# Gyeeta/gyeeta

Hardware: NVIDIA H100
Metric: events/sec aggregated (higher is better)
Workload: dtype u64

## Files before the change

gyeeta_b200/csrc/gysk_device.cuh:

```cuda
#pragma once

#include <cstdint>
#include <cuda_runtime.h>

namespace gysk {

struct HistCell { unsigned long long count; long long sum; };
static constexpr int HIST_CELLS = 16;
static constexpr int HIST_MAX_CELL = 15;

struct alignas(16) TblEntry { unsigned long long key; uint32_t slot1; uint32_t pad; };
static constexpr uint32_t SLOT_INVALID = 0xFFFFFFFFu;

struct Centroid { double mean; unsigned long long weight; };
static constexpr int TD_CAP = 256;

struct alignas(16) Bin { unsigned long long cw; unsigned long long us; };
static constexpr int NBINS = 848;
static constexpr int BIN_CNT_BITS = 27;
static constexpr unsigned long long BIN_CNT_MASK = (1ull << BIN_CNT_BITS) - 1;
static constexpr int HOT_ROW_BINS = 1024, HOT_ROW_WORDS = 2 * HOT_ROW_BINS;
static_assert(NBINS <= HOT_ROW_BINS, "a row holds every bin");
__host__ __device__ __forceinline__ uint32_t hot_word(uint32_t bin) { return ((bin & 31u) << 5) | (bin >> 5); }

struct alignas(8) SlotAux { unsigned long long act_cur, act_last, err_cur, err_last; uint32_t rtt_cur, rtt_last; };

struct alignas(16) SlotBatch { uint32_t minv, maxv, touched, hot; };
struct alignas(8) SlotState { uint8_t state, issue, issue_bits, high_bits; uint32_t nconn_active; };

struct TdHead { unsigned long long total; double minv, maxv; uint32_t n; uint32_t pad; };

struct IdTable
{
	TblEntry	*ent;
	uint32_t	mask;
	uint32_t	max_slots;
	uint32_t	*count;
	unsigned long long *slot_id;
	uint32_t	*slot_host;
	int32_t		*free_n;
	uint32_t	*free_slots;
	unsigned long long *insert_fail;
};
static constexpr unsigned long long KEY_TOMBSTONE = ~0ull;

enum { CTR_IN = 0, CTR_DROPPED, CTR_RESP, CTR_TCP, CTR_TASK, CTR_FOREIGN, CTR_NKEYS, CTR_INSERT_FAIL, CTR_NTOUCHED ,
	CTR_NLONG , CTR_NEVICT, CTR_EVICTED_TOTAL,
	CTR_NHOT , CTR_NHOT_NEXT , CTR_NWINDOW ,
	CTR_NHOSTS , CTR_TASK_NEVICT , CTR_MAX };

static constexpr uint32_t JHASH_GOLDEN = 0x9e3779b9u;
static constexpr uint32_t GY_SEED = 0xceedfeadu;
static constexpr uint32_t FLOW_SEED_A = GY_SEED;
static constexpr uint32_t FLOW_SEED_B = GY_SEED ^ 0x5bd1e995u;

__host__ __device__ __forceinline__ uint32_t jhash_2words(uint32_t a, uint32_t b, uint32_t initval)
{
	uint32_t c = initval;

	a += JHASH_GOLDEN; b += JHASH_GOLDEN;
	a -= b; a -= c; a ^= (c >> 13);
	b -= c; b -= a; b ^= (a << 8);
	c -= a; c -= b; c ^= (b >> 13);
	a -= b; a -= c; a ^= (c >> 12);
	b -= c; b -= a; b ^= (a << 16);
	c -= a; c -= b; c ^= (b >> 5);
	a -= b; a -= c; a ^= (c >> 3);
	b -= c; b -= a; b ^= (a << 10);
	c -= a; c -= b; c ^= (b >> 15);
	return c;
}

__host__ __device__ __forceinline__ uint32_t uint64_hash(unsigned long long key)
{
	return jhash_2words((uint32_t)(key & 0xFFFFFFFFu), (uint32_t)(key >> 32), GY_SEED);
}

__host__ __device__ __forceinline__ uint32_t table_hash(unsigned long long key)
{
	return (uint32_t)((key * 0x9E3779B97F4A7C15ull) >> 32);
}

// ... 99 lines not shown
__device__ __forceinline__ void red_max_s64(long long *p, long long v)
{
	asm volatile("red.global.max.s64 [%0], %1;" :: "l"(p), "l"(v) : "memory");
}

__device__ __forceinline__ void prefetch_l2(const void *p)
{
	asm volatile("prefetch.global.L2 [%0];" :: "l"(p));
}

__device__ __forceinline__ unsigned long long l2_policy_evict_first()
{
	unsigned long long pol;
	asm volatile("createpolicy.fractional.L2::evict_first.b64 %0, 1.0;" : "=l"(pol));
	return pol;
}

__device__ __forceinline__ unsigned long long l2_policy_evict_last()
{
	unsigned long long pol;
	asm volatile("createpolicy.fractional.L2::evict_last.b64 %0, 1.0;" : "=l"(pol));
	return pol;
}

__device__ __forceinline__ void red_add_u64_hint(unsigned long long *p, unsigned long long v, unsigned long long pol)
{
	asm volatile("red.global.add.L2::cache_hint.u64 [%0], %1, %2;" :: "l"(p), "l"(v), "l"(pol) : "memory");
}

__device__ __forceinline__ uint32_t ld_na_hint_u32(const uint32_t *p, unsigned long long pol)
{
	uint32_t v;
	asm volatile("ld.global.L1::no_allocate.L2::cache_hint.u32 %0, [%1], %2;" : "=r"(v) : "l"(p), "l"(pol));
	return v;
}

__device__ __forceinline__ void l2_evict_normal_line(const void *p)
{
	asm volatile("applypriority.global.L2::evict_normal [%0], 128;" :: "l"(p) : "memory");
}

__device__ __forceinline__ uint4 ld_cg_v4(const void *p)
{
	uint4 v;
	asm volatile("ld.global.v4.u32 {%0, %1, %2, %3}, [%4];" : "=r"(v.x), "=r"(v.y), "=r"(v.z), "=r"(v.w) : "l"(p));
	return v;
}

__device__ __forceinline__ uint32_t ld_volatile_u32(const uint32_t *p)
{
	uint32_t v;
	asm volatile("ld.volatile.global.u32 %0, [%1];" : "=r"(v) : "l"(p));
	return v;
}

__device__ __forceinline__ void st_volatile_u32(uint32_t *p, uint32_t v)
{
	asm volatile("st.volatile.global.u32 [%0], %1;" :: "l"(p), "r"(v) : "memory");
}

__device__ __forceinline__ uint4 table_probe_first(const IdTable &t, unsigned long long key, uint32_t &pos)
{
	pos = table_hash(key) & t.mask;
	return ld_cg_v4(&t.ent[pos]);
}

// ... 61 lines not shown
```

gyeeta_b200/csrc/gysk_engine.cu:

```cuda
#include "gysk_engine.h"
#include "gysk_state.cuh"
#include "gysk_summary.cuh"
#include "gysk_wire.h"

using namespace gysk;

namespace {

thread_local std::string g_create_error;
std::atomic<uint64_t> g_engine_uid {1};

}

namespace gysk {

int fail(gysk_engine *e, int code, const char *what, cudaError_t ce)
{
	char buf[512];

	if (ce != cudaSuccess) snprintf(buf, sizeof(buf), "%s: %s", what, cudaGetErrorString(ce));
	else snprintf(buf, sizeof(buf), "%s", what);
	if (e) {
		e->err = buf;
		if (code == GYSK_ERR_CUDA) e->sticky = true;
// ... 508 lines not shown
		A(dalloc(e, &d_q, qtab.size(), false));
		if ((ce = cudaMemcpy(d_q, qtab.data(), qtab.size() * sizeof(double), cudaMemcpyHostToDevice)) != cudaSuccess) { fail(e, GYSK_ERR_CUDA, "qtab", ce); return bail(GYSK_ERR_CUDA); }
		st.td.qtab = d_q; st.td.delta = cfg.td_compression; st.td.pad = 0;
	}
	{
		auto envl = [](const char *name, long dflt) { const char *v = getenv(name); return v ? atol(v) : dflt; };
		long rows = envl("GYSK_HOT_ROWS", 2048);
		if (rows < 0) rows = 0;
		if (rows > 65536) rows = 65536;
		if ((size_t)rows > ns) rows = (long)ns;
		st.hot_cap = (uint32_t)rows;
		st.hot_min = (uint32_t)std::max(1l, envl("GYSK_HOT_MIN", 4096));
		st.hot_max = (uint32_t)std::min<long>(0xFFFFFFFFl, std::max(1l, envl("GYSK_HOT_MAX", 0xFFFFFFFFl)));
		st.hot_bin_max = (uint32_t)std::min<long>(0xFFFFFFFFl, std::max(1l, envl("GYSK_HOT_BIN_MAX", 131072)));
		st.hot_rows = nullptr; st.hot_slot = nullptr;
		if (rows) { A(dalloc(e, &st.hot_rows, (size_t)rows * HOT_ROW_WORDS)); A(dalloc(e, &st.hot_slot, (size_t)rows)); }
	}
	const size_t nsort = sort_keys(cfg);
	tmp.nkeys = nsort;
	tmp.max_tiles = sort_tiles(nsort);
	A(dalloc(e, &tmp.keys_a, nsort, false)); A(dalloc(e, &tmp.keys_b, nsort, false));
	A(dalloc(e, &tmp.tile_status, (size_t)RADIX_MAX * tmp.max_tiles));
	tmp.epoch = &e->sort_epoch;
	A(dalloc(e, &tmp.os_ghist, (size_t)OS_GHIST_WORDS));
	{
		const size_t nmw = (size_t)TD_MERGE_MAX_SMS * TD_MERGE_CTAS_PER_SM * 4;
		const size_t nbrows = batch_rows(cfg);
		A(dalloc(e, &tmp.long_slot, nbrows, false)); A(dalloc(e, &tmp.batch_rows, nbrows * HOT_ROW_WORDS));
		A(dalloc(e, &tmp.items_scratch, nmw * NBINS, false)); A(dalloc(e, &tmp.big_scratch, nmw, false));
		const uint32_t nsm = (uint32_t)prop.multiProcessorCount;
		tmp.rec_cnt_cap = nsm * IngestShape::WARPS * IngestShape::MIN_CTAS;
		tmp.recq_cap = (uint64_t)cfg.max_batch + (uint64_t)tmp.rec_cnt_cap * IngestShape::CHUNK;
		A(dalloc(e, &tmp.recq, (size_t)tmp.recq_cap, false)); A(dalloc(e, &tmp.rec_cnt, (size_t)tmp.rec_cnt_cap, false));
	}
	st.svc_tbl.insert_fail = st.counters + CTR_INSERT_FAIL; st.task_tbl.insert_fail = nullptr;

	for (int k = 0; k < NBUF; ++k) {
		A(dalloc(e, &e->d_events[k], (size_t)cfg.stage_batch, false));
		e->raw_bytes = (size_t)cfg.stage_batch * 32;
		A(dalloc(e, &e->d_raw[k], e->raw_bytes, false));
		if ((ce = cudaEventCreateWithFlags(&e->ev_copied[k], cudaEventDisableTiming)) != cudaSuccess ||
				(ce = cudaEventCreateWithFlags(&e->ev_raw_done[k], cudaEventDisableTiming)) != cudaSuccess ||
				(ce = cudaEventCreateWithFlags(&e->ev_done[k], cudaEventDisableTiming)) != cudaSuccess) {
			fail(e, GYSK_ERR_CUDA, "cudaEventCreate", ce); return bail(GYSK_ERR_CUDA);
		}
	}
	A(dalloc(e, &e->d_qids, (size_t)QCHUNK)); A(halloc(e, &e->h_qids, (size_t)QCHUNK));
	A(halloc(e, &e->h_counters, (size_t)CTR_MAX + 2));
	A(dalloc(e, &e->d_wstage, STAGE_BYTES, false)); A(halloc(e, &e->h_wstage, STAGE_BYTES));
#undef A

	e->kernel_launches += launch_init_slots(st, 0, cfg.max_svcs + 1, 0, cfg.max_tasks, e->stream);
	if ((ce = cudaStreamSynchronize(e->stream)) != cudaSuccess || (ce = cudaGetLastError()) != cudaSuccess) {
		fail(e, GYSK_ERR_CUDA, "engine init", ce); return bail(GYSK_ERR_CUDA);
	}
	*out = e;
	return GYSK_OK;
}

void *gysk_stream(gysk_engine *e) { return e ? (void *)e->stream : nullptr; }

int gysk_profile_enable(gysk_engine *e, int on)
{
	CHECK_ENGINE(e);
	GYSK_ENTER(e, Sync);
	e->profiling = !!on;
// ... 36 lines not shown
	CU(e, cudaMemcpy(&nfree, e->st.svc_tbl.free_n, sizeof(nfree), cudaMemcpyDeviceToHost));
	out->nsvcs = std::min<uint64_t>((uint32_t)e->h_counters[CTR_MAX], e->cfg.max_svcs) - (uint64_t)std::max(nfree, 0);
	out->svcs_evicted = e->evicted_total;
	int32_t tfree = 0;
	if (e->st.task_tbl.free_n) CU(e, cudaMemcpy(&tfree, e->st.task_tbl.free_n, sizeof(tfree), cudaMemcpyDeviceToHost));
	out->ntasks = std::min<uint64_t>((uint32_t)e->h_counters[CTR_MAX + 1], e->cfg.max_tasks) - (uint64_t)std::max(tfree, 0);
	out->batches = e->batches; out->kernel_launches = e->kernel_launches;
	out->wire_msgs_ok = e->wire_ok; out->wire_msgs_bad = e->wire_bad;
	return GYSK_OK;
}

int64_t gysk_hot_rows_in_use(gysk_engine *e)
{
	CHECK_ENGINE(e);
	GYSK_ENTER(e, Sync);
	if (!e->st.hot_rows) return 0;
	unsigned long long n = 0;
	CU(e, cudaMemcpy(&n, e->st.counters + CTR_NHOT_NEXT, sizeof(n), cudaMemcpyDeviceToHost));
	return (int64_t)n;
}

uint32_t gysk_hot_row_word(uint32_t bin)
{
	return bin < (uint32_t)NBINS ? hot_word(bin) : 0xFFFFFFFFu;
}

int64_t gysk_last_batch_keys(gysk_engine *e)
{
	CHECK_ENGINE(e);
	GYSK_ENTER(e, Sync);
	unsigned long long n = 0;
	CU(e, cudaMemcpy(&n, e->st.counters + CTR_NKEYS, sizeof(n), cudaMemcpyDeviceToHost));
	return (int64_t)n;
}

int gysk_register_ids(gysk_engine *e, const uint64_t *ids, uint32_t n, int is_task)
{
	CHECK_ENGINE(e);
	if (!ids && n) return GYSK_ERR_INVAL;
	GYSK_ENTER(e, Drain);
	return staged_read(e, ids, n, QCHUNK, 0, "register",
			[&](const unsigned long long *d_ids, uint32_t, uint32_t m) { return launch_register(e->st, d_ids, m, is_task, e->stream); }, RowsStay {});
}


int gysk_ingest_device(gysk_engine *e, const gysk_event *d_events, uint64_t n)
{
	CHECK_ENGINE(e);
	if (!d_events && n) return GYSK_ERR_INVAL;
	GYSK_ENTER(e, Submit);
	for (uint64_t off = 0; off < n; off += e->cfg.max_batch) {
		const uint64_t m = std::min<uint64_t>(e->cfg.max_batch, n - off);
		if (int rc = process_device_batch(e, d_events + off, m, nullptr)) return rc;
	}
	return GYSK_OK;
}

int gysk_ingest_pinned(gysk_engine *e, const gysk_event *pinned, uint64_t n)
{
	CHECK_ENGINE(e);
	if (!pinned && n) return GYSK_ERR_INVAL;
	GYSK_ENTER(e, Drain);
	return append_chunk(e, pinned, n);
}

}
// ... 1166 lines not shown
```

gyeeta_b200/csrc/gysk_kernels.cu:

```cuda
#include "gysk_kernels.cuh"
#include "gysk_state.cuh"
#include "gysk_summary.cuh"

#include <cfloat>
#include <climits>
#include <cmath>
#include <algorithm>
#include <type_traits>
#include <cstdlib>
#include <cstring>

namespace gysk {

static constexpr int KEY_GROUP_SHIFT = 30;
static constexpr int KEY_SLOT_SHIFT = KEY_GROUP_SHIFT + TD_CODE_BITS;
__device__ __forceinline__ uint32_t key_usec(unsigned long long k) { return (uint32_t)k & 0x3FFFFFFFu; }
__device__ __forceinline__ uint32_t key_slot(unsigned long long k) { return (uint32_t)(k >> KEY_SLOT_SHIFT); }
__device__ __forceinline__ uint32_t key_bin(unsigned long long k) { return (uint32_t)(k >> KEY_GROUP_SHIFT) & ((1u << TD_CODE_BITS) - 1u); }

static constexpr int KEY_DIGIT_MAX = 8;
static constexpr int KEY_SLOT_BITS_MAX = 24;
static constexpr int KEY_PASSES_MAX = (TD_CODE_BITS + KEY_SLOT_BITS_MAX + KEY_DIGIT_MAX - 1) / KEY_DIGIT_MAX;
static_assert(KEY_PASSES_MAX <= OS_MAX_PASSES, "a RESP plan fits a SortPlan");
struct SortPlan { int np; int shift[OS_MAX_PASSES]; int bits[OS_MAX_PASSES]; };
// ... 119 lines not shown
__device__ __forceinline__ uint32_t hll_peek(const uint8_t *regs, uint32_t idx)
{
	return __ldca(reinterpret_cast<const uint32_t *>(regs) + (idx >> 2));
}

__device__ __forceinline__ void hll_raise(uint8_t *regs, uint32_t idx, uint32_t rank, uint32_t w)
{
	uint32_t *wp = reinterpret_cast<uint32_t *>(regs) + (idx >> 2);
	const uint32_t sh = (idx & 3u) * 8u;

	while (((w >> sh) & 0xFFu) < rank) {
		const uint32_t nw = (w & ~(0xFFu << sh)) | (rank << sh);
		const uint32_t old = atomicCAS(wp, w, nw);
		if (old == w) break;
		w = old;
	}
}

__device__ __forceinline__ void hll_update(uint8_t *regs, uint32_t idx, uint32_t rank)
{
	hll_raise(regs, idx, rank, hll_peek(regs, idx));
}

struct alignas(16) IngestRec { uint32_t slot; uint32_t value; unsigned long long flow_key; };
static_assert(sizeof(IngestRec) == 16, "IngestRec travels as one uint4");

__device__ __forceinline__ IngestRec ld_rec(const IngestRec *p)
{
	const uint4 v = __ldcs(reinterpret_cast<const uint4 *>(p));
	IngestRec r; r.slot = v.x; r.value = v.y; r.flow_key = ((unsigned long long)v.w << 32) | v.z;
	return r;
}

template <typename HotTable>
__device__ __forceinline__ void drain_tcp_recs(const DevState &st, HotTable &hot, const IngestRec *q, uint32_t m, int lane,
		unsigned long long pol_hll, unsigned long long pol_cms, int exp)
{
	for (uint32_t i = lane; i < ((m + 31u) & ~31u); i += 32) {
		const bool act = i < m;
		uint32_t cell = 0, idx = 0, rank = 0, hw = 0; int kb = 0;
		if (act) {
			const IngestRec r = ld_rec(q + i);
			uint32_t h1, h2;
			flow_hashes(r.flow_key, h1, h2);
			if (!(exp & 32)) {
				hll_idx_rank2(h1, h2, st.hll_p, idx, rank);
				hw = ld_na_hint_u32(reinterpret_cast<const uint32_t *>(st.hll + ((size_t)r.slot << st.hll_p)) + (idx >> 2), pol_hll);
			}
			const unsigned long long inc = cms_increment(r.value);
			if (!(exp & 16))
				for (uint32_t row = 0; row < st.cms_depth; ++row)
					red_add_u64_hint(st.cms_cur + ((size_t)row << st.cms_log2w) + cms_index2(h1, h2, row, st.cms_wmask), inc, pol_cms);
			cell = r.slot;
			kb = (int)(r.value >> 10);
		}
		cell_add(st, hot, act, cell, kb);
		if (act && !(exp & 32)) hll_raise(st.hll + ((size_t)cell << st.hll_p), idx, rank, hw);
	}
}

template <int ADMIT, typename HotTable>
__device__ __forceinline__ void drain_task_group(const DevState &st, HotTable &hot, const IngestRec &r, bool act, int exp, uint32_t &sink)
{
	const int d[3] = {(int)r.value, (int)(uint32_t)r.flow_key, (int)(uint32_t)(r.flow_key >> 32)};
	uint32_t cell[3];
#pragma unroll
	for (uint32_t h = 0; h < 3; ++h) {
		const uint32_t b = h == 0 ? (uint32_t)bucket_hash_1_3000(d[h]) : (uint32_t)bucket_duration(d[h]);
		cell[h] = CELL_TASK | (r.slot * 3u * HIST_CELLS + h * HIST_CELLS + b);
	}
#pragma unroll
	for (int h = 0; h < 3; ++h) {
		if (exp & 128) sink += act ? cell[h] : 0u;
		else cell_add<ADMIT>(st, hot, act, cell[h], d[h], !(exp & 64));
	}
}


struct IngestShared
{
	static constexpr int KQ_CAP = 192, KQ_FLUSH = KQ_CAP - IngestShape::CHUNK;
	static constexpr int RQ_CAP = 32 + IngestShape::CHUNK;
	static constexpr int DH = 1 << KEY_DIGIT_MAX;
	struct Warp { unsigned long long kq[KQ_CAP]; IngestRec tcp[RQ_CAP], task[RQ_CAP]; };
	Warp		w[IngestShape::WARPS];
	uint32_t	dhist[KEY_PASSES_MAX][DH];
};

__global__ void __launch_bounds__(IngestShape::WARPS * 32, IngestShape::MIN_CTAS) ingest_kernel(DevState st, const gysk_event *__restrict__ ev, uint64_t n,
// ... 162 lines not shown
		if (nk > (uint32_t)IngestShared::KQ_FLUSH) flush_keys();
	}
	if (ntcp) { drain_tcp(ntcp); t_tcp += ntcp; }
	if (ntask) { drain_task(ntask); t_task += ntask; }
	if (nk) flush_keys();
	if (lane == 0) rec_cnt[gwarp] = make_uint2((uint32_t)t_tcp, (uint32_t)t_task);

	__syncthreads();
	for (int i = threadIdx.x; i < plan.np * DH; i += WARPS * 32) {
		const uint32_t c = (&S.dhist[0][0])[i];
		if (c) atomicAdd(ghist + (i / DH) * RADIX_MAX + (i % DH), c);
	}

	c_in = __reduce_add_sync(0xffffffffu, c_in);
	c_foreign = __reduce_add_sync(0xffffffffu, c_foreign);
	const unsigned long long t_resp = __reduce_add_sync(0xffffffffu, n_resp);
	t_tcp += __reduce_add_sync(0xffffffffu, n_active);
	if (lane == 0) {
		if (c_in) atomicAdd(st.counters + CTR_IN, (unsigned long long)c_in);
		if (c_foreign) atomicAdd(st.counters + CTR_FOREIGN, (unsigned long long)c_foreign);
		if (t_resp) atomicAdd(st.counters + CTR_RESP, t_resp);
		if (t_tcp) atomicAdd(st.counters + CTR_TCP, t_tcp);
		if (t_task) atomicAdd(st.counters + CTR_TASK, t_task);
		const unsigned long long q = t_resp + t_tcp + t_task;
		if (c_in != q) atomicAdd(st.counters + CTR_DROPPED, (unsigned long long)c_in - q);
	}
}

template <bool TASK> struct DrainShape;
template <> struct DrainShape<false> { static constexpr int WARPS = 8, HOT_BITS = 12, ADMIT = 2; };
template <> struct DrainShape<true> { static constexpr int WARPS = 16, HOT_BITS = 13, ADMIT = 1; };

template <bool TASK>
__global__ void __launch_bounds__(DrainShape<TASK>::WARPS * 32) drain_kernel(DevState st, const uint4 *__restrict__ q, const uint2 *__restrict__ cnt, RecRegions rr, int exp)
{
	constexpr int WARPS = DrainShape<TASK>::WARPS;
	using DrainHot = HotTableT<DrainShape<TASK>::HOT_BITS>;
	if (TASK) {
		const size_t lines = ((size_t)st.cms_depth << st.cms_log2w) * sizeof(unsigned long long) / 128u;
		for (size_t i = (size_t)blockIdx.x * blockDim.x + threadIdx.x; i < lines; i += (size_t)gridDim.x * blockDim.x)
			l2_evict_normal_line(reinterpret_cast<const char *>(st.cms_cur) + i * 128u);
	}
	const unsigned long long pol_hll = TASK ? 0 : l2_policy_evict_first(), pol_cms = TASK ? 0 : l2_policy_evict_last();
	extern __shared__ __align__(16) unsigned char drain_smem[];
	DrainHot &hot = *reinterpret_cast<DrainHot *>(drain_smem);
	uint32_t *rstart = reinterpret_cast<uint32_t *>(drain_smem + sizeof(DrainHot));
	__shared__ uint32_t wsum[WARPS];
	const int lane = threadIdx.x & 31, wid = threadIdx.x >> 5;
	for (int i = threadIdx.x; i < DrainHot::N; i += WARPS * 32) { hot.tag[i] = 0; hot.count[i] = 0; hot.sum[i] = 0; hot.vmax[i] = INT_MIN; }

	const uint32_t nreg = rr.nwarps, per = (nreg + WARPS * 32 - 1) / (WARPS * 32), r0 = threadIdx.x * per;
	const uint32_t r1 = min(r0 + per, nreg);
	uint32_t s = 0;
	for (uint32_t r = r0; r < r1; ++r) {
		const uint32_t c = TASK ? cnt[r].y : cnt[r].x;
		rstart[r] = c; s += (c + 31u) >> 5;
	}
	uint32_t incl = s;
#pragma unroll
	for (int off = 1; off < 32; off <<= 1) { const uint32_t t = __shfl_up_sync(0xffffffffu, incl, off); if (lane >= off) incl += t; }
	if (lane == 31) wsum[wid] = incl;
	__syncthreads();
	uint32_t g0 = incl - s, ngroups = 0;
#pragma unroll
	for (int w = 0; w < WARPS; ++w) { if (w < wid) g0 += wsum[w]; ngroups += wsum[w]; }
	for (uint32_t r = r0; r < r1; ++r) { const uint32_t c = rstart[r]; rstart[r] = (g0 << 5) | (c & 31u); g0 += (c + 31u) >> 5; }
	if (threadIdx.x == 0) rstart[nreg] = ngroups << 5;
	__syncthreads();

	const uint32_t gw = blockIdx.x * WARPS + wid, nw = gridDim.x * WARPS;
	const uint32_t gbeg = (uint32_t)((unsigned long long)ngroups * gw / nw), gend = (uint32_t)((unsigned long long)ngroups * (gw + 1) / nw);
	const IngestRec *recs = reinterpret_cast<const IngestRec *>(q);
	uint32_t r = 0;
	for (uint32_t hi = nreg; r < hi; ) { const uint32_t mid = (r + hi + 1) >> 1; if ((rstart[mid] >> 5) <= gbeg) r = mid; else hi = mid - 1; }
	auto locate = [&](uint32_t g, uint32_t &off, uint32_t &m) {
		while ((rstart[r + 1] >> 5) <= g) ++r;
		const uint32_t first = rstart[r] >> 5, tail = rstart[r] & 31u;
		off = (g - first) * 32u;
		m = (g + 1 == rstart[r + 1] >> 5 && tail) ? tail : 32u;
	};
	if (TASK) {
		uint32_t sink = 0;
		auto fetch = [&](uint32_t g, uint32_t &m) {
			uint32_t off;
			locate(g, off, m);
			IngestRec rec {0u, 0u, 0ull};
			if ((uint32_t)lane < m) rec = ld_rec(recs + (unsigned long long)r * rr.cap + (rr.cap - 1 - off - lane));
			return rec;
		};
		uint32_t m = 0;
		IngestRec next = gbeg < gend ? fetch(gbeg, m) : IngestRec {0u, 0u, 0ull};
		for (uint32_t g = gbeg; g < gend; ++g) {
			const IngestRec cur = next;
			const bool act = (uint32_t)lane < m;
			if (g + 1 < gend) next = fetch(g + 1, m);
			drain_task_group<DrainShape<TASK>::ADMIT>(st, hot, cur, act, exp, sink);
		}
		if (sink == 1u) atomicAdd(&hot.count[0], 1u);
	}
	else {
		for (uint32_t g = gbeg; g < gend; ++g) {
			uint32_t off, m;
			locate(g, off, m);
			drain_tcp_recs(st, hot, recs + (unsigned long long)r * rr.cap + off, m, lane, pol_hll, pol_cms, exp);
		}
	}

	__syncthreads();
	for (int i = threadIdx.x; i < DrainHot::N; i += WARPS * 32) {
		if (hot.tag[i] && hot.count[i]) cell_add_global(st, hot.tag[i] - 1, hot.count[i], hot.sum[i], hot.vmax[i]);
	}
}

static constexpr int OS_THREADS = 256;
static constexpr int OS_WARPS = OS_THREADS / 32;
static constexpr int OS_KPT = SORT_TILE / OS_THREADS;
static constexpr uint32_t OS_FLAG_AGG = 1u << 30, OS_FLAG_PREFIX = 2u << 30, OS_COUNT_MASK = (1u << 30) - 1u;

__device__ __forceinline__ unsigned long long ld_volatile_u64(const unsigned long long *p)
{
	unsigned long long v;
	asm volatile("ld.volatile.global.u64 %0, [%1];" : "=l"(v) : "l"(p));
	return v;
}
__device__ __forceinline__ void st_volatile_u64(unsigned long long *p, unsigned long long v)
{
	asm volatile("st.volatile.global.u64 [%0], %1;" :: "l"(p), "l"(v) : "memory");
}

template <int copies, int stride>
__global__ void __launch_bounds__(512) os_hist_kernel(const unsigned long long *__restrict__ keys, const unsigned long long *__restrict__ d_n, SortPlan P,
		uint32_t *__restrict__ ghist )
{
	extern __shared__ __align__(16) unsigned char osh_smem[];
	uint32_t *h = reinterpret_cast<uint32_t *>(osh_smem);
	const int copy = threadIdx.x & (copies - 1);
	constexpr int pstride = copies * stride;
// ... 1110 lines not shown
		P.shift[P.np] = at;
		P.bits[P.np] = std::min(wide-- > 0 ? 9 : 8, hi - at);
	}
	return 0;
}

int launch_ingest(const DevState &st, const SortTemp &tmp, const gysk_event *d_ev, uint64_t n, uint32_t max_svcs, RecRegions &rr, cudaStream_t s)
{
	if (!n) return 0;
	const int dev = current_device();
	SortPlan plan {};
	if (key_sort_plan(max_svcs, plan) < 0) return -1;
	if (st.hot_rows) cudaMemcpyAsync(st.counters + CTR_NHOT, st.counters + CTR_NHOT_NEXT, sizeof(unsigned long long), cudaMemcpyDeviceToDevice, s);
	cudaMemsetAsync(st.counters + CTR_NKEYS, 0, sizeof(unsigned long long), s);
	cudaMemsetAsync(tmp.os_ghist, 0, OS_GHIST_WORDS * sizeof(uint32_t), s);
	constexpr int WARPS = IngestShape::WARPS, CHUNK = IngestShape::CHUNK;
	static bool attr_set[MAX_DEVICES] = {};
	if (!attr_set[dev]) {
		cudaFuncSetAttribute(ingest_kernel, cudaFuncAttributeMaxDynamicSharedMemorySize, (int)sizeof(IngestShared));
		attr_set[dev] = true;
	}
	const uint64_t want = (n + (uint64_t)CHUNK * WARPS - 1) / ((uint64_t)CHUNK * WARPS);
	const uint64_t full = (uint64_t)sm_count(dev) * IngestShape::MIN_CTAS;
	const uint32_t grid = (uint32_t)(want < full ? want : full);
	const uint64_t nchunks = (n + CHUNK - 1) / CHUNK;
	rr.nwarps = grid * WARPS;
	rr.cap = (nchunks + rr.nwarps - 1) / rr.nwarps * CHUNK;
	if (rr.nwarps > tmp.rec_cnt_cap || (uint64_t)rr.nwarps * rr.cap > tmp.recq_cap) return -1;
	ingest_kernel<<<grid, WARPS * 32, sizeof(IngestShared), s>>>(st, d_ev, n, tmp.keys_a, tmp.os_ghist, plan, tmp.recq, tmp.rec_cnt, exp_ablate());
	return 1;
}

template <bool TASK>
static void launch_drain_pass(const DevState &st, const SortTemp &tmp, const RecRegions &rr, uint64_t n_events, int exp, int dev, cudaStream_t s)
{
	constexpr int WARPS = DrainShape<TASK>::WARPS;
	constexpr size_t HOT_BYTES = sizeof(HotTableT<DrainShape<TASK>::HOT_BITS>);
	static int per_sm[MAX_DEVICES] = {};
	if (!per_sm[dev]) {
		const size_t smem_max = HOT_BYTES + ((size_t)tmp.rec_cnt_cap + 1) * sizeof(uint32_t);
		cudaFuncSetAttribute(drain_kernel<TASK>, cudaFuncAttributeMaxDynamicSharedMemorySize, (int)smem_max);
		int b = 0;
		cudaOccupancyMaxActiveBlocksPerMultiprocessor(&b, drain_kernel<TASK>, WARPS * 32, smem_max);
		per_sm[dev] = b > 0 ? b : 1;
	}
	const uint64_t want = (n_events + WARPS * 32 - 1) / (WARPS * 32);
	const uint64_t full = (uint64_t)sm_count(dev) * per_sm[dev];
	const size_t smem = HOT_BYTES + ((size_t)rr.nwarps + 1) * sizeof(uint32_t);
	drain_kernel<TASK><<<(uint32_t)(want < full ? want : full), WARPS * 32, smem, s>>>(st, tmp.recq, tmp.rec_cnt, rr, exp);
}

int launch_drains(const DevState &st, const SortTemp &tmp, const RecRegions &rr, uint64_t n_events, cudaStream_t s)
{
	if (!n_events) return 0;
	const int dev = current_device();
	const int exp = exp_ablate();
	int launches = 0;
	if (!(exp & 4)) { launch_drain_pass<false>(st, tmp, rr, n_events, exp, dev, s); launches++; }
	if (!(exp & 8)) { launch_drain_pass<true>(st, tmp, rr, n_events, exp, dev, s); launches++; }
	return launches;
}

static void os_set_attrs(int dev)
{
	static bool attr_set[MAX_DEVICES] = {};
	if (attr_set[dev]) return;
	cudaFuncSetAttribute(os_pass_kernel<6>, cudaFuncAttributeMaxDynamicSharedMemorySize, (int)sizeof(OneSweepSharedT<6>));
	cudaFuncSetAttribute(os_pass_kernel<7>, cudaFuncAttributeMaxDynamicSharedMemorySize, (int)sizeof(OneSweepSharedT<7>));
	cudaFuncSetAttribute(os_pass_kernel<8>, cudaFuncAttributeMaxDynamicSharedMemorySize, (int)sizeof(OneSweepSharedT<8>));
	cudaFuncSetAttribute(os_pass_kernel<9>, cudaFuncAttributeMaxDynamicSharedMemorySize, (int)sizeof(OneSweepSharedT<9>));
	cudaFuncSetAttribute(os_hist_kernel<8, 257>, cudaFuncAttributeMaxDynamicSharedMemorySize, OS_MAX_PASSES * 8 * 257 * (int)sizeof(uint32_t));
	cudaFuncSetAttribute(os_hist_kernel<4, 513>, cudaFuncAttributeMaxDynamicSharedMemorySize, OS_MAX_PASSES * 4 * 513 * (int)sizeof(uint32_t));
	attr_set[dev] = true;
}

static uint32_t next_epoch(const SortTemp &tmp, uint32_t max_tiles, cudaStream_t s)
{
	uint32_t e = ++*tmp.epoch;
	if (e == 0) {
		cudaMemsetAsync(tmp.tile_status, 0, (size_t)max_tiles * RADIX_MAX * sizeof(unsigned long long), s);
		e = ++*tmp.epoch;
	}
	return e;
}

static int launch_sort_passes(const SortPlan &P, const SortTemp &tmp, const unsigned long long *d_n, uint32_t ntiles, int *which, cudaStream_t s)
{
	unsigned long long *bufs[2] = { tmp.keys_a, tmp.keys_b };
	const uint32_t grid = std::min<uint32_t>(ntiles, (uint32_t)sm_count(current_device()) * 4u);
	int w = 0;

	for (int p = 0; p < P.np; ++p, w ^= 1) {
// ... 280 lines not shown
```

gyeeta_b200/csrc/gysk_kernels.cuh:

```cuda
#pragma once

#include "gysk_device.cuh"
#include "gysk_tdigest.cuh"
#include "../../include/gysketch.h"

#include <climits>

namespace gysk {

static constexpr int NLEVELS = 2;
static constexpr int NSLOTS = 10;

struct LevelRing
{
	HistCell		*ring;
	uint32_t		stride;
	uint32_t		live[NLEVELS];
	uint32_t		cur[NLEVELS];
	uint32_t		fresh;

	__host__ __device__ __forceinline__ HistCell *row(int l, uint32_t k, uint32_t slot) const
	{
		return ring + (((size_t)l * NSLOTS + k) * stride + slot) * HIST_CELLS;
	}
// ... 29 lines not shown
	SlotBatch		*slot_batch;
	unsigned long long	*hot_rows;
	uint32_t		*hot_slot;
	uint32_t		hot_cap, hot_min, hot_max, hot_bin_max;
	SlotAux			*slot_aux;
	HistCell		*qps_hist, *act_hist;
	SlotState		*slot_state;
	uint8_t			*hll;
	Centroid		*td_cent;
	TdHead			*td_head;
	HistCell		*task_hist;
	HistCell		*task_prev, *task_last;
	unsigned long long	*task_slot_id;
	uint32_t		*task_slot_host;
	uint32_t		*task_last_active;
	uint32_t		*task_evict_list;
	unsigned long long	*task_evict_ids;
	unsigned long long	*cms_cur, *cms_last;
	unsigned long long	*cms_ring, *cms_5min;
	uint32_t		cms_depth, cms_wmask, cms_log2w, hll_p;
	uint32_t		rank, world, auto_register;
	double			td_delta;
	TdParams		td;
	unsigned long long	*counters;
};

__device__ __forceinline__ bool svc_live(const DevState &st, uint32_t slot) { return st.slot_id[slot] != 0; }
__device__ __forceinline__ bool svc_evaluated(const DevState &st, uint32_t slot, uint32_t active_mark) { return st.slot_last_active[slot] == active_mark; }
__device__ __forceinline__ bool svc_issue(const DevState &st, uint32_t slot, uint32_t active_mark)
{
	return svc_evaluated(st, slot, active_mark) && (st.slot_state[slot].issue_bits & 1u);
}

struct SortTemp
{
	unsigned long long	*keys_a, *keys_b;
	uint64_t		nkeys;
	unsigned long long	*tile_status;
	uint32_t		*epoch;
	uint32_t		*os_ghist;
	uint32_t		*touched;
	uint4			*segs;
	uint32_t		*long_slot;
	unsigned long long	*batch_rows;
	Centroid		*items_scratch;
	TdWorkBig		*big_scratch;
	uint4			*recq;
	uint2			*rec_cnt;
	uint64_t		recq_cap;
	uint32_t		rec_cnt_cap;
	uint32_t		max_tiles;
};

struct RecRegions { uint32_t nwarps; uint64_t cap; };

struct IngestShape { static constexpr int WARPS = 8, MIN_CTAS = 3, EPT = 2, CHUNK = 32 * EPT; };

struct SvcRaw
{
	unsigned long long	id;
	int32_t			found;
	uint32_t		slot;
	HistCell		cur[HIST_CELLS], last[HIST_CELLS], all[HIST_CELLS];
	HistCell		lvl[2][HIST_CELLS];
	unsigned long long	conn_cur, conn_last, conn_all_cnt, conn_all_kb;
	uint32_t		bm_cur[HIST_CELLS], bm_last[HIST_CELLS];
	uint32_t		hll_hist[64];
	TdHead			td;
	SlotAux			aux;
	SlotState		sst;
	HistCell		qps[HIST_CELLS], act[HIST_CELLS];
	Centroid		cent[TD_CAP];
};

struct TaskRaw
{
	unsigned long long	id;
	int32_t			found;
	uint32_t		slot;
	HistCell		h[3][HIST_CELLS];
};

static constexpr int SORT_TILE = 4096;
// ... 40 lines not shown
```

gyeeta_b200/engine.py:

```python
import ctypes as C
import os

import numpy as np

HERE = os.path.dirname(os.path.abspath(__file__))
LIB_PATH = os.path.join(HERE, "libgysketch.so")

EVENT_DTYPE = np.dtype([("svc_id", "<u8"), ("flow_key", "<u8"), ("value", "<u4"), ("host_idx", "<u4"),
                        ("tsec", "<u4"), ("type", "<u2"), ("flags", "<u2")], align=True)
assert EVENT_DTYPE.itemsize == 32
SERIAL_DTYPE = np.dtype([("count", "<u8"), ("sum", "<i8")])
FLOW_EST_DTYPE = np.dtype([("flow_key", "<u8"), ("count", "<u4"), ("kbytes", "<u4")])

EV_CONNECT, EV_ACCEPT, EV_CLOSE_CLI, EV_CLOSE_SER, EV_RESP, EV_TASK, EV_ACTIVE = 1, 2, 3, 4, 5, 6, 7
EVF_CLI_ERROR, EVF_SER_ERROR = 1, 2
HIST_RESP_CUR, HIST_RESP_LAST, HIST_RESP_ALL, HIST_TASK_CPU_PCT, HIST_TASK_CPU_DELAY, HIST_TASK_BLKIO_DELAY, HIST_RESP_5MIN, HIST_RESP_5DAY, HIST_QPS, HIST_ACTIVE_CONN = range(10)
STATE_IDLE, STATE_GOOD, STATE_OK, STATE_BAD, STATE_SEVERE, STATE_DOWN = range(6)
ISSUE_NONE, ISSUE_LISTENER_TASKS, ISSUE_QPS_HIGH, ISSUE_ACTIVE_CONN_HIGH, ISSUE_SERVER_ERRORS, ISSUE_OS_CPU, ISSUE_OS_MEMORY, ISSUE_DEPENDENT, ISSUE_UNKNOWN = range(9)
TOPN_QPS, TOPN_CONNS, TOPN_NET, TOPN_ISSUE, TOPN_ACTIVE = range(5)
RAW_EVENT32, RAW_TCP_IPV4_EVENT, RAW_TCP_IPV4_RESP, RAW_TCP_IPV6_EVENT, RAW_TCP_IPV6_RESP, RAW_API_TRAN, RAW_RESP16, RAW_TCP24, RAW_TASK24 = range(9)
RESP16_DTYPE = np.dtype([("svc_id", "<u8"), ("usec", "<u4"), ("host_idx", "<u2"), ("cli_port", "u1"), ("flags", "u1")])
TCP24_DTYPE = np.dtype([("svc_id", "<u8"), ("flow_key", "<u8"), ("bytes", "<u4"), ("host_idx", "<u2"), ("type", "u1"), ("pad", "u1")])
TASK24_DTYPE = np.dtype([("aggr_task_id", "<u8"), ("cpu_pct", "<u4"), ("cpu_delay_msec", "<u4"), ("blkio_delay_msec", "<u4"), ("host_idx", "<u2"), ("pad", "<u2")])
PROC_SAMPLE_DTYPE = np.dtype([("aggr_task_id", "<u8"), ("pid", "<i4"), ("cpu_pct", "<f4"), ("rss_mb", "<u4"), ("cpu_delay_msec", "<u4"),
# ... 156 lines not shown
    s, t = C.c_uint64(), C.c_uint64()
    rc = L.gysk_slot_bytes(C.byref(cfg), C.byref(s), C.byref(t))
    if rc:
        raise GyskError(rc, "gysk_slot_bytes")
    return s.value, t.value


class BufferDesc(C.Structure):
    _fields_ = [("name", C.c_char_p), ("dptr", C.c_void_p), ("nbytes", C.c_uint64), ("redop", C.c_int32), ("pad", C.c_int32)]


_lib = None


def load_library(path=None):
    global _lib
    if _lib is not None and path is None:
        return _lib
    path = path or LIB_PATH
    if not os.path.exists(path):
        raise GyskError(-19, f"{path} is missing: build it with `python -m gyeeta_b200.build` "
                             "(CUDA library is the product; no CPU fallback exists)")
    L = C.CDLL(path)
    vp, u32, u64, i32 = C.c_void_p, C.c_uint32, C.c_uint64, C.c_int
    sig = {
        "gysk_abi_version": (i32, []),
        "gysk_config_default": (None, [vp]),
        "gysk_create": (i32, [vp, vp]),
        "gysk_destroy": (None, [vp]),
        "gysk_last_error": (C.c_char_p, [vp]),
        "gysk_get_stats": (i32, [vp, vp]),
        "gysk_hot_rows_in_use": (C.c_int64, [vp]),
        "gysk_last_batch_keys": (C.c_int64, [vp]),
        "gysk_register_ids": (i32, [vp, vp, u32, i32]),
        "gysk_ingest": (i32, [vp, vp, u32, u32, vp, u32, vp]),
        "gysk_ingest_msg": (i32, [vp, vp, u32, vp, u32]),
        "gysk_ingest_raw": (i32, [vp, vp, u32, u32, vp, u32]),
        "gysk_ingest_pinned": (i32, [vp, vp, u64]),
        "gysk_ingest_device": (i32, [vp, vp, u64]),
        "gysk_sync": (i32, [vp]),
        "gysk_flush": (i32, [vp, u32]),
        "gysk_evicted_ids": (i32, [vp, vp, u32, vp]),
        "gysk_evicted_task_ids": (i32, [vp, vp, u32, vp]),
        "gysk_task_evict_count": (i32, [vp, vp]),
        "gysk_query_svcs": (i32, [vp, vp, u32, vp]),
        "gysk_query_flows": (i32, [vp, vp, u32, i32, vp]),
        "gysk_query_window": (i32, [vp, C.c_int32, u32, vp, u32, vp]),
        "gysk_query_window_hosts": (i32, [vp, C.c_int32, u32, vp, vp, u32, vp]),
        "gysk_query_tasks": (i32, [vp, vp, u32, vp]),
        "gysk_query_task_window": (i32, [vp, C.c_int32, u32, vp, u32, vp]),
        "gysk_query_host_summary": (i32, [vp, u32, vp]),
        "gysk_topn_svcs": (i32, [vp, i32, C.c_int32, u32, vp, vp]),
        "gysk_topn_tasks": (i32, [vp, i32, u32, vp, vp]),
        "gysk_topn_host": (i32, [vp, i32, C.c_int32, u32, vp, vp]),
        "gysk_query_cluster_state": (i32, [vp, vp, u32, vp]),
        "gysk_export_hist": (i32, [vp, u64, i32, vp, vp, vp]),
        "gysk_export_task_hist": (i32, [vp, u64, i32, vp, vp, vp]),
        "gysk_export_hll": (i32, [vp, u64, vp]),
        "gysk_export_conn_bitmap": (i32, [vp, u64, i32, vp, vp]),
        "gysk_export_tdigest": (i32, [vp, u64, vp, vp, u32, vp, vp, vp]),
        "gysk_query_quantiles": (i32, [vp, u64, vp, u32, vp]),
        "gysk_tdigest_to_pgtext": (i32, [vp, vp, u32, u32, vp, u32]),
        "gysk_encode_listener_state": (i32, [vp, u32, vp, u32, vp, vp]),
        "gysk_export_tdigest_pgtext": (i32, [vp, u64, vp, u32]),
        "gysk_export_cms": (i32, [vp, i32, vp]),
        "gysk_hist_nbuckets": (i32, [i32]),
# ... 164 lines not shown
    def grow(self, max_svcs=None, max_tasks=None):
        cap = self.capacity()
        ms = cap["max_svcs"] if max_svcs is None else max_svcs
        mt = cap["max_tasks"] if max_tasks is None else max_tasks
        self._chk(self.L.gysk_grow(self.h, ms, mt))
        self.cfg.max_svcs, self.cfg.max_tasks = ms, mt

    def set_auto_grow(self, max_svcs_limit=0, max_tasks_limit=0):
        self._chk(self.L.gysk_set_auto_grow(self.h, max_svcs_limit, max_tasks_limit))

    def capacity(self):
        c = Capacity()
        self._chk(self.L.gysk_capacity_info(self.h, C.byref(c)))
        self.cfg.max_svcs, self.cfg.max_tasks = c.max_svcs, c.max_tasks
        return c.asdict()

    def stats(self):
        s = Stats()
        self._chk(self.L.gysk_get_stats(self.h, C.byref(s)))
        return s.asdict()

    def hot_rows_in_use(self):
        n = self.L.gysk_hot_rows_in_use(self.h)
        if n < 0:
            self._chk(int(n))
        return int(n)

    def last_batch_keys(self):
        n = self.L.gysk_last_batch_keys(self.h)
        if n < 0:
            self._chk(int(n))
        return int(n)

    def query_svcs(self, ids):
        ids = np.ascontiguousarray(ids, dtype=np.uint64)
        out = (SvcSummary * len(ids))()
        self._chk(self.L.gysk_query_svcs(self.h, _p(ids), len(ids), out))
        return [o.asdict() for o in out]

    def listener_state_records(self, ids):
        ids = np.ascontiguousarray(ids, dtype=np.uint64)
        out = (SvcSummary * len(ids))()
        self._chk(self.L.gysk_query_svcs(self.h, _p(ids), len(ids), out))
        buf = C.create_string_buffer(88 * 512)
        nrecs, nbytes = C.c_uint32(), C.c_uint32()
        self._chk(self.L.gysk_encode_listener_state(out, len(ids), buf, len(buf), C.byref(nrecs), C.byref(nbytes)))
        return nrecs.value, buf.raw[: nbytes.value]

    def _window(self, fn, row_type, args, active_only, cap):
        flags = WINDOW_ACTIVE_ONLY if active_only else 0
        n = C.c_uint32()
        if cap is None:
            self._chk(fn(self.h, *args, flags, None, 0, C.byref(n)))
            cap = n.value
        out = (row_type * max(cap, 1))()
        self._chk(fn(self.h, *args, flags, out if cap else None, cap, C.byref(n)))
        return out[: min(cap, n.value)], n.value

    def query_window(self, host_idx=-1, active_only=False, cap=None):
        return self._window(self.L.gysk_query_window, SvcSummary, (host_idx,), active_only, cap)

    def query_window_hosts(self, host_idx=-1, active_only=False, cap=None):
        flags = WINDOW_ACTIVE_ONLY if active_only else 0
        n = C.c_uint32()
        if cap is None:
            self._chk(self.L.gysk_query_window_hosts(self.h, host_idx, flags, None, None, 0, C.byref(n)))
# ... 292 lines not shown
```

include/gysketch.h:

```cpp
#ifndef GYSKETCH_H
#define GYSKETCH_H

#include <stdint.h>
#include <stddef.h>

#ifdef __cplusplus
extern "C" {
#endif

#define GYSK_ABI_VERSION		2

#define GYSK_OK				0
#define GYSK_ERR_INVAL			(-22)
#define GYSK_ERR_NOMEM			(-12)
#define GYSK_ERR_NOENT			(-2)
#define GYSK_ERR_NOSPC			(-28)
#define GYSK_ERR_NODEV			(-19)
#define GYSK_ERR_CUDA			(-5)
#define GYSK_ERR_NOTSUP			(-95)

enum {
	GYSK_EV_CONNECT		= 1,
	GYSK_EV_ACCEPT		= 2,
	GYSK_EV_CLOSE_CLI	= 3,
// ... 214 lines not shown

typedef struct gysk_stats
{
	uint64_t	events_in;
	uint64_t	events_dropped;
	uint64_t	events_resp, events_tcp, events_task;
	uint64_t	nsvcs, ntasks;
	uint64_t	batches;
	uint64_t	kernel_launches;
	uint64_t	wire_msgs_ok, wire_msgs_bad;
	uint64_t	svcs_evicted;
} gysk_stats;

enum { GYSK_RED_SUM_U64 = 0, GYSK_RED_MAX_U8 = 1, GYSK_RED_MAX_I64 = 2 };
typedef struct gysk_buffer_desc
{
	const char	*name;
	void		*dptr;
	uint64_t	nbytes;
	int32_t		redop;
	int32_t		pad;
} gysk_buffer_desc;

int		gysk_abi_version(void);
void		gysk_config_default(gysk_config *cfg);
int		gysk_create(const gysk_config *cfg, gysk_engine **out);
void		gysk_destroy(gysk_engine *e);
const char *	gysk_last_error(gysk_engine *e);
int		gysk_get_stats(gysk_engine *e, gysk_stats *out);
int64_t		gysk_hot_rows_in_use(gysk_engine *e);
#define GYSK_HOT_ROW_BINS	1024u
uint32_t	gysk_hot_row_word(uint32_t bin);
int64_t		gysk_last_batch_keys(gysk_engine *e);

int		gysk_grow(gysk_engine *e, uint32_t max_svcs, uint32_t max_tasks);

int		gysk_set_auto_grow(gysk_engine *e, uint32_t max_svcs_limit, uint32_t max_tasks_limit);

typedef struct gysk_capacity
{
	uint32_t	max_svcs, max_tasks;
	uint32_t	svcs_in_use, tasks_in_use;
	uint32_t	ngrows, pad;
	uint64_t	device_bytes;
} gysk_capacity;
int		gysk_capacity_info(gysk_engine *e, gysk_capacity *out);

int		gysk_slot_bytes(const gysk_config *cfg, uint64_t *svc_slot_bytes, uint64_t *task_slot_bytes);

int		gysk_register_ids(gysk_engine *e, const uint64_t *ids, uint32_t n, int is_task);

int		gysk_ingest(gysk_engine *e, const uint8_t host_id[16], uint32_t host_idx, uint32_t subtype,
				void *recs, uint32_t nevents, const void *endptr);
int		gysk_ingest_msg(gysk_engine *e, const uint8_t host_id[16], uint32_t host_idx, void *comm_header_msg, uint32_t msglen);
int		gysk_ingest_raw(gysk_engine *e, const uint8_t host_id[16], uint32_t host_idx, uint32_t kind,
				const void *events, uint32_t nevents);
int		gysk_ingest_pinned(gysk_engine *e, const gysk_event *pinned_events, uint64_t nevents);
int		gysk_ingest_device(gysk_engine *e, const gysk_event *d_events, uint64_t nevents);
int		gysk_export_task_hist(gysk_engine *e, uint64_t aggr_task_id, int which, gysk_hist_serial out[GYSK_HIST_MAX_BUCKETS],
				uint64_t *total_count, int64_t *max_val);
int		gysk_sync(gysk_engine *e);
int		gysk_flush(gysk_engine *e, uint32_t tsec);
int		gysk_evicted_ids(gysk_engine *e, uint64_t *out, uint32_t cap, uint32_t *n);

int		gysk_evicted_task_ids(gysk_engine *e, uint64_t *out, uint32_t cap, uint32_t *n);
int		gysk_task_evict_count(gysk_engine *e, uint64_t *total);
// ... 160 lines not shown
```

Baseline: 12.16 billion.

## Pre-aggregate TCP flow CMS increments in a hash table before sketch update

Instead of issuing depth-many CMS atomic adds per TCP record, the non-task drain now accumulates increments per flow key in an open-addressed hash table. The task drain pass then sweeps the table, applies one set of CMS adds per distinct flow, and clears the entries. Records that fail to find a slot within the probe limit fall back to direct CMS updates, counted in a new counter. This cuts CMS atomic traffic when flows repeat, at the cost of extra CAS probes, a table sweep, and making the task pass mandatory.

```diff
diff --git a/gyeeta_b200/csrc/gysk_device.cuh b/gyeeta_b200/csrc/gysk_device.cuh
--- a/gyeeta_b200/csrc/gysk_device.cuh
+++ b/gyeeta_b200/csrc/gysk_device.cuh
@@ -47,7 +47,8 @@
 enum { CTR_IN = 0, CTR_DROPPED, CTR_RESP, CTR_TCP, CTR_TASK, CTR_FOREIGN, CTR_NKEYS, CTR_INSERT_FAIL, CTR_NTOUCHED ,
 	CTR_NLONG , CTR_NEVICT, CTR_EVICTED_TOTAL,
 	CTR_NHOT , CTR_NHOT_NEXT , CTR_NWINDOW ,
-	CTR_NHOSTS , CTR_TASK_NEVICT , CTR_MAX };
+	CTR_NHOSTS , CTR_TASK_NEVICT ,
+	CTR_FLOW_DIRECT , CTR_MAX };
 
 static constexpr uint32_t JHASH_GOLDEN = 0x9e3779b9u;
 static constexpr uint32_t GY_SEED = 0xceedfeadu;
@@ -213,6 +214,13 @@
 {
 	uint32_t v;
 	asm volatile("ld.global.L1::no_allocate.L2::cache_hint.u32 %0, [%1], %2;" : "=r"(v) : "l"(p), "l"(pol));
+	return v;
+}
+
+__device__ __forceinline__ unsigned long long ld_cg_hint_u64(const unsigned long long *p, unsigned long long pol)
+{
+	unsigned long long v;
+	asm volatile("ld.global.cg.L2::cache_hint.u64 %0, [%1], %2;" : "=l"(v) : "l"(p), "l"(pol));
 	return v;
 }
 
diff --git a/gyeeta_b200/csrc/gysk_engine.cu b/gyeeta_b200/csrc/gysk_engine.cu
--- a/gyeeta_b200/csrc/gysk_engine.cu
+++ b/gyeeta_b200/csrc/gysk_engine.cu
@@ -564,6 +564,8 @@
 		tmp.rec_cnt_cap = nsm * IngestShape::WARPS * IngestShape::MIN_CTAS;
 		tmp.recq_cap = (uint64_t)cfg.max_batch + (uint64_t)tmp.rec_cnt_cap * IngestShape::CHUNK;
 		A(dalloc(e, &tmp.recq, (size_t)tmp.recq_cap, false)); A(dalloc(e, &tmp.rec_cnt, (size_t)tmp.rec_cnt_cap, false));
+		tmp.flow_cap = std::min<uint32_t>(FLOW_ENT_MAX, pow2_at_least(2ull * cfg.max_batch));
+		A(dalloc(e, &tmp.flow, (size_t)tmp.flow_cap));
 	}
 	st.svc_tbl.insert_fail = st.counters + CTR_INSERT_FAIL; st.task_tbl.insert_fail = nullptr;
 
@@ -666,6 +668,24 @@
 	unsigned long long n = 0;
 	CU(e, cudaMemcpy(&n, e->st.counters + CTR_NKEYS, sizeof(n), cudaMemcpyDeviceToHost));
 	return (int64_t)n;
+}
+
+int64_t gysk_last_batch_flow_direct(gysk_engine *e)
+{
+	CHECK_ENGINE(e);
+	GYSK_ENTER(e, Sync);
+	unsigned long long n = 0;
+	CU(e, cudaMemcpy(&n, e->st.counters + CTR_FLOW_DIRECT, sizeof(n), cudaMemcpyDeviceToHost));
+	return (int64_t)n;
+}
+
+int64_t gysk_flow_table_used(gysk_engine *e)
+{
+	CHECK_ENGINE(e);
+	GYSK_ENTER(e, Sync);
+	std::vector<FlowEnt> t(e->tmp.flow_cap);
+	CU(e, cudaMemcpy(t.data(), e->tmp.flow, t.size() * sizeof(FlowEnt), cudaMemcpyDeviceToHost));
+	return (int64_t)std::count_if(t.begin(), t.end(), [](const FlowEnt &f) { return f.key || f.inc; });
 }
 
 int gysk_register_ids(gysk_engine *e, const uint64_t *ids, uint32_t n, int is_task)
diff --git a/gyeeta_b200/csrc/gysk_kernels.cu b/gyeeta_b200/csrc/gysk_kernels.cu
--- a/gyeeta_b200/csrc/gysk_kernels.cu
+++ b/gyeeta_b200/csrc/gysk_kernels.cu
@@ -175,13 +175,33 @@
 	return r;
 }
 
+__device__ __forceinline__ void flow_add(const DevState &st, const FlowTable &ft, unsigned long long key, uint32_t pos, unsigned long long k,
+		unsigned long long inc, unsigned long long pol_last)
+{
+	if (key) {
+		for (uint32_t p = 0; ; ) {
+			if (k == 0) k = atomicCAS(&ft.ent[pos].key, 0ull, key);
+			if (k == 0 || k == key) { red_add_u64_hint(&ft.ent[pos].inc, inc, pol_last); return; }
+			if (++p == FLOW_PROBES) break;
+			pos = (pos + 1) & ft.mask;
+			k = ld_cg_hint_u64(&ft.ent[pos].key, pol_last);
+		}
+	}
+	const uint32_t am = __activemask();
+	if ((threadIdx.x & 31) == __ffs(am) - 1) atomicAdd(st.counters + CTR_FLOW_DIRECT, (unsigned long long)__popc(am));
+	const uint32_t h1 = (uint32_t)key, h2 = (uint32_t)(key >> 32);
+	for (uint32_t row = 0; row < st.cms_depth; ++row)
+		red_add_u64(st.cms_cur + ((size_t)row << st.cms_log2w) + cms_index2(h1, h2, row, st.cms_wmask), inc);
+}
+
 template <typename HotTable>
-__device__ __forceinline__ void drain_tcp_recs(const DevState &st, HotTable &hot, const IngestRec *q, uint32_t m, int lane,
-		unsigned long long pol_hll, unsigned long long pol_cms, int exp)
+__device__ __forceinline__ void drain_tcp_recs(const DevState &st, const FlowTable &ft, HotTable &hot, const IngestRec *q, uint32_t m,
+		int lane, unsigned long long pol_hll, unsigned long long pol_last, int exp)
 {
 	for (uint32_t i = lane; i < ((m + 31u) & ~31u); i += 32) {
 		const bool act = i < m;
-		uint32_t cell = 0, idx = 0, rank = 0, hw = 0; int kb = 0;
+		uint32_t cell = 0, idx = 0, rank = 0, hw = 0, pos = 0; int kb = 0;
+		unsigned long long key = 0, inc = 0, k = 0;
 		if (act) {
 			const IngestRec r = ld_rec(q + i);
 			uint32_t h1, h2;
@@ -190,14 +210,15 @@
 				hll_idx_rank2(h1, h2, st.hll_p, idx, rank);
 				hw = ld_na_hint_u32(reinterpret_cast<const uint32_t *>(st.hll + ((size_t)r.slot << st.hll_p)) + (idx >> 2), pol_hll);
 			}
-			const unsigned long long inc = cms_increment(r.value);
-			if (!(exp & 16))
-				for (uint32_t row = 0; row < st.cms_depth; ++row)
-					red_add_u64_hint(st.cms_cur + ((size_t)row << st.cms_log2w) + cms_index2(h1, h2, row, st.cms_wmask), inc, pol_cms);
+			key = ((unsigned long long)h2 << 32) | h1;
+			inc = cms_increment(r.value);
+			pos = table_hash(key) & ft.mask;
+			if (key && !(exp & 16)) k = ld_cg_hint_u64(&ft.ent[pos].key, pol_last);
 			cell = r.slot;
 			kb = (int)(r.value >> 10);
 		}
 		cell_add(st, hot, act, cell, kb);
+		if (act && !(exp & 16)) flow_add(st, ft, key, pos, k, inc, pol_last);
 		if (act && !(exp & 32)) hll_raise(st.hll + ((size_t)cell << st.hll_p), idx, rank, hw);
 	}
 }
@@ -426,16 +447,31 @@
 template <> struct DrainShape<true> { static constexpr int WARPS = 16, HOT_BITS = 13, ADMIT = 1; };
 
 template <bool TASK>
-__global__ void __launch_bounds__(DrainShape<TASK>::WARPS * 32) drain_kernel(DevState st, const uint4 *__restrict__ q, const uint2 *__restrict__ cnt, RecRegions rr, int exp)
+__global__ void __launch_bounds__(DrainShape<TASK>::WARPS * 32) drain_kernel(DevState st, FlowTable ft, const uint4 *__restrict__ q, const uint2 *__restrict__ cnt,
+		RecRegions rr, int exp)
 {
 	constexpr int WARPS = DrainShape<TASK>::WARPS;
 	using DrainHot = HotTableT<DrainShape<TASK>::HOT_BITS>;
 	if (TASK) {
-		const size_t lines = ((size_t)st.cms_depth << st.cms_log2w) * sizeof(unsigned long long) / 128u;
-		for (size_t i = (size_t)blockIdx.x * blockDim.x + threadIdx.x; i < lines; i += (size_t)gridDim.x * blockDim.x)
-			l2_evict_normal_line(reinterpret_cast<const char *>(st.cms_cur) + i * 128u);
-	}
-	const unsigned long long pol_hll = TASK ? 0 : l2_policy_evict_first(), pol_cms = TASK ? 0 : l2_policy_evict_last();
+		const uint32_t stride = gridDim.x * blockDim.x;
+		for (uint32_t i0 = blockIdx.x * blockDim.x + threadIdx.x; i0 <= ft.mask; i0 += FLOW_SWEEP * stride) {
+			FlowEnt f[FLOW_SWEEP];
+#pragma unroll
+			for (uint32_t u = 0; u < FLOW_SWEEP; ++u) if (i0 + u * stride <= ft.mask) f[u] = ft.ent[i0 + u * stride]; else f[u] = FlowEnt {0ull, 0ull};
+#pragma unroll
+			for (uint32_t u = 0; u < FLOW_SWEEP; ++u) {
+				const uint32_t i = i0 + u * stride;
+				if (f[u].key) {
+					const uint32_t h1 = (uint32_t)f[u].key, h2 = (uint32_t)(f[u].key >> 32);
+					for (uint32_t row = 0; row < st.cms_depth; ++row)
+						red_add_u64(st.cms_cur + ((size_t)row << st.cms_log2w) + cms_index2(h1, h2, row, st.cms_wmask), f[u].inc);
+					ft.ent[i] = FlowEnt {0ull, 0ull};
+				}
+				if (i <= ft.mask && !(i & 7u)) l2_evict_normal_line(ft.ent + i);
+			}
+		}
+	}
+	const unsigned long long pol_hll = TASK ? 0 : l2_policy_evict_first(), pol_last = TASK ? 0 : l2_policy_evict_last();
 	extern __shared__ __align__(16) unsigned char drain_smem[];
 	DrainHot &hot = *reinterpret_cast<DrainHot *>(drain_smem);
 	uint32_t *rstart = reinterpret_cast<uint32_t *>(drain_smem + sizeof(DrainHot));
@@ -463,7 +499,8 @@
 	__syncthreads();
 
 	const uint32_t gw = blockIdx.x * WARPS + wid, nw = gridDim.x * WARPS;
-	const uint32_t gbeg = (uint32_t)((unsigned long long)ngroups * gw / nw), gend = (uint32_t)((unsigned long long)ngroups * (gw + 1) / nw);
+	const uint32_t gbeg = (uint32_t)((unsigned long long)ngroups * gw / nw);
+	const uint32_t gend = (TASK && (exp & 8)) ? gbeg : (uint32_t)((unsigned long long)ngroups * (gw + 1) / nw);
 	const IngestRec *recs = reinterpret_cast<const IngestRec *>(q);
 	uint32_t r = 0;
 	for (uint32_t hi = nreg; r < hi; ) { const uint32_t mid = (r + hi + 1) >> 1; if ((rstart[mid] >> 5) <= gbeg) r = mid; else hi = mid - 1; }
@@ -496,7 +533,7 @@
 		for (uint32_t g = gbeg; g < gend; ++g) {
 			uint32_t off, m;
 			locate(g, off, m);
-			drain_tcp_recs(st, hot, recs + (unsigned long long)r * rr.cap + off, m, lane, pol_hll, pol_cms, exp);
+			drain_tcp_recs(st, ft, hot, recs + (unsigned long long)r * rr.cap + off, m, lane, pol_hll, pol_last, exp);
 		}
 	}
 
@@ -1673,7 +1710,8 @@
 }
 
 template <bool TASK>
-static void launch_drain_pass(const DevState &st, const SortTemp &tmp, const RecRegions &rr, uint64_t n_events, int exp, int dev, cudaStream_t s)
+static void launch_drain_pass(const DevState &st, const FlowTable &ft, const SortTemp &tmp, const RecRegions &rr, uint64_t n_events, int exp, int dev,
+		cudaStream_t s)
 {
 	constexpr int WARPS = DrainShape<TASK>::WARPS;
 	constexpr size_t HOT_BYTES = sizeof(HotTableT<DrainShape<TASK>::HOT_BITS>);
@@ -1688,7 +1726,7 @@
 	const uint64_t want = (n_events + WARPS * 32 - 1) / (WARPS * 32);
 	const uint64_t full = (uint64_t)sm_count(dev) * per_sm[dev];
 	const size_t smem = HOT_BYTES + ((size_t)rr.nwarps + 1) * sizeof(uint32_t);
-	drain_kernel<TASK><<<(uint32_t)(want < full ? want : full), WARPS * 32, smem, s>>>(st, tmp.recq, tmp.rec_cnt, rr, exp);
+	drain_kernel<TASK><<<(uint32_t)(want < full ? want : full), WARPS * 32, smem, s>>>(st, ft, tmp.recq, tmp.rec_cnt, rr, exp);
 }
 
 int launch_drains(const DevState &st, const SortTemp &tmp, const RecRegions &rr, uint64_t n_events, cudaStream_t s)
@@ -1696,9 +1734,13 @@
 	if (!n_events) return 0;
 	const int dev = current_device();
 	const int exp = exp_ablate();
+	uint32_t n = 16;
+	while (n < tmp.flow_cap && n < 2 * n_events) n <<= 1;
+	const FlowTable ft {tmp.flow, n - 1u};
+	cudaMemsetAsync(st.counters + CTR_FLOW_DIRECT, 0, sizeof(unsigned long long), s);
 	int launches = 0;
-	if (!(exp & 4)) { launch_drain_pass<false>(st, tmp, rr, n_events, exp, dev, s); launches++; }
-	if (!(exp & 8)) { launch_drain_pass<true>(st, tmp, rr, n_events, exp, dev, s); launches++; }
+	if (!(exp & 4)) { launch_drain_pass<false>(st, ft, tmp, rr, n_events, exp, dev, s); launches++; }
+	launch_drain_pass<true>(st, ft, tmp, rr, n_events, exp, dev, s); launches++;
 	return launches;
 }
 
diff --git a/gyeeta_b200/csrc/gysk_kernels.cuh b/gyeeta_b200/csrc/gysk_kernels.cuh
--- a/gyeeta_b200/csrc/gysk_kernels.cuh
+++ b/gyeeta_b200/csrc/gysk_kernels.cuh
@@ -85,6 +85,12 @@
 	return svc_evaluated(st, slot, active_mark) && (st.slot_state[slot].issue_bits & 1u);
 }
 
+struct alignas(16) FlowEnt { unsigned long long key, inc; };
+struct FlowTable { FlowEnt *ent; uint32_t mask; };
+static constexpr uint32_t FLOW_PROBES = 16;
+static constexpr uint32_t FLOW_ENT_MAX = 1u << 21;
+static constexpr uint32_t FLOW_SWEEP = 4;
+
 struct SortTemp
 {
 	unsigned long long	*keys_a, *keys_b;
@@ -102,6 +108,8 @@
 	uint2			*rec_cnt;
 	uint64_t		recq_cap;
 	uint32_t		rec_cnt_cap;
+	FlowEnt			*flow;
+	uint32_t		flow_cap;
 	uint32_t		max_tiles;
 };
 
diff --git a/gyeeta_b200/engine.py b/gyeeta_b200/engine.py
--- a/gyeeta_b200/engine.py
+++ b/gyeeta_b200/engine.py
@@ -212,6 +212,8 @@
         "gysk_get_stats": (i32, [vp, vp]),
         "gysk_hot_rows_in_use": (C.c_int64, [vp]),
         "gysk_last_batch_keys": (C.c_int64, [vp]),
+        "gysk_last_batch_flow_direct": (C.c_int64, [vp]),
+        "gysk_flow_table_used": (C.c_int64, [vp]),
         "gysk_register_ids": (i32, [vp, vp, u32, i32]),
         "gysk_ingest": (i32, [vp, vp, u32, u32, vp, u32, vp]),
         "gysk_ingest_msg": (i32, [vp, vp, u32, vp, u32]),
@@ -442,6 +444,18 @@
             self._chk(int(n))
         return int(n)
 
+    def last_batch_flow_direct(self):
+        n = self.L.gysk_last_batch_flow_direct(self.h)
+        if n < 0:
+            self._chk(int(n))
+        return int(n)
+
+    def flow_table_used(self):
+        n = self.L.gysk_flow_table_used(self.h)
+        if n < 0:
+            self._chk(int(n))
+        return int(n)
+
     def query_svcs(self, ids):
         ids = np.ascontiguousarray(ids, dtype=np.uint64)
         out = (SvcSummary * len(ids))()
diff --git a/include/gysketch.h b/include/gysketch.h
--- a/include/gysketch.h
+++ b/include/gysketch.h
@@ -270,6 +270,8 @@
 #define GYSK_HOT_ROW_BINS	1024u
 uint32_t	gysk_hot_row_word(uint32_t bin);
 int64_t		gysk_last_batch_keys(gysk_engine *e);
+int64_t		gysk_last_batch_flow_direct(gysk_engine *e);
+int64_t		gysk_flow_table_used(gysk_engine *e);
 
 int		gysk_grow(gysk_engine *e, uint32_t max_svcs, uint32_t max_tasks);
 
```

Result: faster. 12.78 billion (median of 6 runs) (+5.1%).
